# JinPLu/VeloxSeg

Hardware: AMD Instinct MI355X
Metric: training patches/s on 128^3 2-mod volumes (fwd+loss+bwd+allreduce+AdamW) (higher is better)
Workload: dtype f32

## Files before the change

### include/veloxseg_hip.h

```cpp
#ifndef VELOXSEG_HIP_H
#define VELOXSEG_HIP_H

#ifdef __cplusplus
extern "C" {
#endif

#define VX_ABI_VERSION 1

int vx_abi_version(void);
const char* vx_last_error(void);

int vx_conv3d_fwd(const float* x, const float* x2, int C1, const float* w, const float* bias, float* y,
                  int B, int Cin, int Di, int Hi, int Wi, int Cout, int K, int S, int P, int G, int ps, void* stream);
int vx_conv3d_bwd_data(const float* dy, const float* w, const float* bias_like, float* dx, float* dx2, int C1,
                       int B, int Cin, int Di, int Hi, int Wi, int Cout, int K, int S, int P, int G, int ps,
                       int accumulate, void* stream);
int vx_conv3d_bwd_weight(const float* x, const float* x2, int C1, const float* dy, float* dw, float* db,
                         int B, int Cin, int Di, int Hi, int Wi, int Cout, int K, int S, int P, int G, int ps, void* stream);

int vx_conv3d_bwd_weight_tiled(const float* x, const float* x2, int C1, const float* dy, float* dw, float* db,
                               int B, int Cin, int Di, int Hi, int Wi, int Cout, int K, int S, int P, int G, int ps, void* stream);
int vx_down_wgrad_ws_floats(int B, int Cin, int Di, int Hi, int Wi, int Cout);
int vx_down_wgrad_mfma(const float* x, const float* dy, float* dw, float* db, float* ws, long ws_floats,
                       int B, int Cin, int Di, int Hi, int Wi, int Cout, void* stream);
// ... 88 lines not shown
                 unsigned long long site2, float p2, int h16, void* stream);

int vx_jlc_tz_ok(int C, int G, int D, int H, int W);
int vx_jlc_tz_ntiles(int C, int G, int D, int H, int W);
int vx_jlc_tz_img_floats(int C, int G);
int vx_jlc_tz_set_pieces(int ns);
int vx_jlc_tz_set_min_voxels(long v);
int vx_jlc_tz_pieces(void);
int vx_jlc_tz_set_debug(int mask);
int vx_jlc_tz_prep(const float* w1, const float* w3, const float* w5, float* img, int C, int G, void* stream);
int vx_jlc_tz_fwd(const float* x, const float* img, const float* b1, const float* b3, const float* b5, float* y1, float* y3, float* y5, double* part,
                  int B, int C, int G, int D, int H, int W, void* stream);
int vx_jlc_tz_bwd(const float* g1, const float* g3, const float* g5, const float* img, const float* w1, const float* d_o, float* dx,
                  int B, int C, int G, int D, int H, int W, void* stream);
int vx_jlc_cl_ok(int C, int G, int D, int H, int W);
int vx_jlc_cl_ntiles(int C, int G, int D, int H, int W);
int vx_jlc_cl_img_floats(int C, int G);
int vx_jlc_cl_set_enabled(int on);
int vx_jlc_cl_prep(const float* w1, const float* w3, const float* w5, float* img, int C, int G, void* stream);
int vx_jlc_cl_fwd(const float* x, const float* img, const float* b1, const float* b3, const float* b5, float* y1, float* y3, float* y5, double* part,
                  int B, int C, int G, int D, int H, int W, void* stream);
int vx_jlc_cl_bwd(const float* g1, const float* g3, const float* g5, const float* img, const float* d_o, float* dx, int B, int C, int G, int D, int H, int W,
                  void* stream);
int vx_jlc_wgrad_tz_ok(int C, int G, int D, int H, int W);
int vx_jlc_wgrad_tz_set_min_voxels(long v);
int vx_jlc_wgrad_tz_set_blocks(int n);
int vx_jlc_wgrad_tz_set_spec(int on);
int vx_jlc_wgrad_tz_set_f16(int on);
int vx_jlc_wgrad_tz(const float* x, const float* g1, const float* g3, const float* g5, float* dw1, float* dw3, float* dw5, int B, int C, int G, int D, int H, int W,
                    void* stream);
int vx_jlc_tz_img_floats_ns(int C, int G, int pieces);
int vx_jlc_tz_prep_ns(const float* w1, const float* w3, const float* w5, float* img, int C, int G, int pieces, void* stream);
int vx_jlc_tz_fwd_ns(const float* x, const float* img, const float* b1, const float* b3, const float* b5, float* y1, float* y3, float* y5, double* part,
                     int B, int C, int G, int D, int H, int W, int pieces, void* stream);
int vx_jlc_tz_bwd_ns(const float* g1, const float* g3, const float* g5, const float* img, const float* w1, const float* d_o, float* dx,
                     int B, int C, int G, int D, int H, int W, int pieces, void* stream);
int vx_jlc_wgrad_tz_ns(const float* x, const float* g1, const float* g3, const float* g5, float* dw1, float* dw3, float* dw5, int B, int C, int G, int D, int H, int W,
                       int pieces, void* stream);
int vx_jlc_tz_fwd_h(const float* x, const float* img, const float* b1, const float* b3, const float* b5, void* y1, void* y3, void* y5, double* part,
                    int B, int C, int G, int D, int H, int W, int pieces, int h16, void* stream);
int vx_jlc_tz_bwd_h(const void* g1, const void* g3, const void* g5, const float* img, const float* w1, const void* d_o, float* dx,
                    int B, int C, int G, int D, int H, int W, int pieces, int h16, void* stream);
int vx_jlc_wgrad_tz_h(const float* x, const void* g1, const void* g3, const void* g5, float* dw1, float* dw3, float* dw5, int B, int C, int G, int D, int H, int W,
                      int pieces, int h16, void* stream);

int vx_in_stats(const float* x, float* stats, double* part_ws, long BC, long V, float eps, void* stream);
// ... 239 lines not shown
```

### veloxseg_amd/csrc/_vxops.cpp

```cpp
#include <torch/extension.h>
#include <torch/csrc/autograd/custom_function.h>
#include <torch/custom_class.h>
#include <torch/library.h>
#include <c10/hip/HIPStream.h>
#include <ATen/hip/impl/HIPStreamMasqueradingAsCUDA.h>
#include <ATen/hip/impl/HIPGuardImplMasqueradingAsCUDA.h>
#include <hip/hip_runtime_api.h>
#include <algorithm>
#include <map>
#include <unordered_map>
#include <tuple>
#include <functional>
#include <type_traits>
#include <memory>
#include <vector>
#include <map>
#include <tuple>
#include "../../include/veloxseg_hip.h"

using at::Tensor;
typedef c10::optional<Tensor> OptT;

namespace {

// ... 482 lines not shown
    return out;
}

void axpy_bwd_impl(AxpyState& st, const Tensor& dout_in, bool need_x_in, Tensor& dx, Tensor& dz, void* stream) {
    Tensor dout = contig(dout_in);
    const bool need_x = st.has_x && need_x_in;
    if (st.p == 0.0 && (st.alpha == 1.0 || !need_x)) { if (need_x) dx = dout; dz = dout; return; }
    if (need_x) dx = st.alpha == 1.0 ? dout : at::empty_like(dout);
    dz = st.p == 0.0 ? dout : at::empty_like(dout);
    VX(vx_axpy_drop_bwd, fp(dout), (need_x && st.alpha != 1.0) ? mp(dx) : nullptr, st.p > 0 ? mp(dz) : nullptr, (float)st.alpha, dout.numel(), st.rs,
                         (unsigned long long)st.site, (float)st.p, stream);
}

inline Tensor sum3(const Tensor& a, const Tensor& b, const Tensor& c, void* stream) {
    Tensor ac = contig(a), bc = contig(b), cc = c.defined() ? contig(c) : Tensor();
    Tensor out = at::empty_like(ac);
    VX(vx_add, fp(ac), fp(bc), fp(cc), mp(out), ac.numel(), stream);
    return out;
}

struct JLCFusedState {
    Tensor x, y, o, stats_y, stats_o;
    bool img_cl = false;
    int tz_pieces = 0;
    Tensor img;
    Tensor w1, w3, w5, b1, b3, b5, l1w, l1b, l2w, l2b;
    int B = 0, C = 0, G = 0, D = 0, H = 0, W = 0, R = 0, nch = 0;
    bool tile = false;
    bool h16 = false;
    double p = 0; int64_t site = 0; const void* rs = nullptr;
};
struct JLCState {
    std::vector<ConvState> convs;
    INState in1, in2;
    ConvState c1, c2;
    GeluState g;
    AxpyState r;
    bool fused = false;
    bool blk = false;
    JLCFusedState f;
};

struct FFNState {
    LNState ln;
    ConvState c1, c2;
    GeluState g;
// ... 369 lines not shown
    return 0;
}
static std::pair<Tensor, std::shared_ptr<JLCState>> jlc_fwd_f(const Tensor& x, const std::vector<Tensor>& ws, const std::vector<Tensor>& bs, int G, const Tensor& l1w, const Tensor& l1b, const Tensor& l2w,
                        const Tensor& l2b, double p, int64_t site, int64_t rs, int64_t stream) {
        auto st = std::make_shared<JLCState>();
        void* s_ = sp(stream);
        const int n = (int)ws.size();
        if (F.fuse_blocks && n == 3 && x.dim() == 5 && ws[0].size(2) == 1 && ws[1].size(2) == 3 && ws[2].size(2) == 5) {
            const int B = x.size(0), C = x.size(1), D = x.size(2), H = x.size(3), W = x.size(4), R = l1w.size(0);
            const long V = (long)D * H * W;
            const bool mlp_ok = vx_mlp_supported(C, R, V) && C < F.tile_min_c, tile_ok = !mlp_ok && F.jlc_tile && V % 4 == 0 && vx_inmlp_ok(C, R, V);
            if ((C / G) % 4 == 0 && (mlp_ok || tile_ok) && bs[0].defined() && bs[1].defined() && bs[2].defined()) {
                check_in(x, "jlc");
                JLCFusedState& f = st->f;
                st->blk = true;
                f.x = contig(x);
                f.w1 = ws[0]; f.w3 = ws[1]; f.w5 = ws[2]; f.b1 = bs[0]; f.b3 = bs[1]; f.b5 = bs[2]; f.l1w = l1w; f.l1b = l1b; f.l2w = l2w; f.l2b = l2b;
                f.B = B; f.C = C; f.G = G; f.D = D; f.H = H; f.W = W; f.R = R; f.p = p; f.site = site; f.rs = p > 0 ? sp(rs) : nullptr;
                const long BC = (long)B * C;
                const bool tz = F.jlc_tz && vx_jlc_tz_ok(C, G, D, H, W);
                const bool cl = !tz && F.jlc_tz && vx_jlc_cl_ok(C, G, D, H, W);
                const int nty = tz ? vx_jlc_tz_ntiles(C, G, D, H, W) : cl ? vx_jlc_cl_ntiles(C, G, D, H, W) : vx_jlc_ntiles(B, C, G, D, H, W);
                TORCH_CHECK(nty > 0, "vx_jlc_ntiles failed");
                f.nch = vx_jlc_nchunks(BC, V);
                auto dopt = f.x.options().dtype(at::kDouble);
                Tensor part_y = at::empty({3, BC, nty, 2}, dopt), part_o = at::empty({BC, (long)f.nch, 2}, dopt);
                f.tile = tile_ok;
                f.tz_pieces = tz ? vx_jlc_tz_pieces() : 0;
                f.h16 = F.act_bf16 && tz && !tile_ok && f.tz_pieces == 1 && F.jlc_wg_tz && vx_jlc_wgrad_tz_ok(C, G, D, H, W) == 1 && V > 64;
                auto iopt = f.h16 ? f.x.options().dtype(at::kBFloat16) : f.x.options();
                const long esz = f.h16 ? 2 : 4;
                f.y = at::empty({3, B, C, D, H, W}, iopt);
                char* yp = (char*)f.y.data_ptr();
                const long n1 = BC * V;
                void *y1 = yp, *y3 = yp + esz * n1, *y5 = yp + 2 * esz * n1;
                bool pre = false;
                {
                    auto it = JLC_PRE.find(f.w1.data_ptr());
                    if (it != JLC_PRE.end()) {
                        const JlcPreImg& q = it->second;
                        pre = q.C == C && q.G == G && ((tz && q.kind == 1 && q.pieces == f.tz_pieces) || (cl && q.kind == 2));
                        if (pre && q.keep) pre = q.epoch == WEIGHTS_EPOCH && q.ver == jlc_wver(f.w1, f.w3, f.w5);
                        if (pre) f.img = q.img;
                        if (!(pre && q.keep)) JLC_PRE.erase(it);
                    }
                }
                if (tz) {
                    if (!pre) {
                        f.img = at::empty({(long)vx_jlc_tz_img_floats_ns(C, G, f.tz_pieces)}, f.x.options());
                        VX(vx_jlc_tz_prep_ns, fp(f.w1), fp(f.w3), fp(f.w5), mp(f.img), C, G, f.tz_pieces, s_);
                    }
                    VX(vx_jlc_tz_fwd_h, fp(f.x), fp(f.img), fp(f.b1), fp(f.b3), fp(f.b5), y1, y3, y5, part_y.data_ptr<double>(), B, C, G, D, H, W, f.tz_pieces, (int)f.h16, s_);
                } else if (cl) {
                    f.img_cl = true;
                    if (!pre) {
                        f.img = at::empty({(long)vx_jlc_cl_img_floats(C, G)}, f.x.options());
                        VX(vx_jlc_cl_prep, fp(f.w1), fp(f.w3), fp(f.w5), mp(f.img), C, G, s_);
                    }
                    VX(vx_jlc_cl_fwd, fp(f.x), fp(f.img), fp(f.b1), fp(f.b3), fp(f.b5), (float*)y1, (float*)y3, (float*)y5, part_y.data_ptr<double>(), B, C, G, D, H, W, s_);
                } else
                VX(vx_jlc_conv_fwd, fp(f.x), fp(f.w1), fp(f.w3), fp(f.w5), fp(f.b1), fp(f.b3), fp(f.b5), (float*)y1, (float*)y3, (float*)y5, part_y.data_ptr<double>(), B, C, G, D, H, W, s_);
                f.stats_y = at::empty({3, BC, 2}, f.x.options());
                f.stats_o = at::empty({BC, 2}, f.x.options());
                f.o = at::empty(f.x.sizes(), iopt);
                VX(vx_jlc_mid_fwd_h, fp(f.x), (const void*)y1, (const void*)y3, (const void*)y5, part_y.data_ptr<double>(), nty, mp(f.stats_y), f.o.data_ptr(), part_o.data_ptr<double>(), BC, V, (float)F.in_eps, (int)f.h16, s_);
                Tensor out = at::empty_like(f.x);
                if (tile_ok) VX(vx_inmlp_fwd, fp(f.o), part_o.data_ptr<double>(), f.nch, mp(f.stats_o), fp(l1w), fp(l1b), fp(l2w), fp(l2b), mp(out), B, C, R, V, (float)F.in_eps,
                                f.rs, (unsigned long long)site, (float)p, s_);
                else
                VX(vx_mlp_fwd_h, (const void*)f.o.data_ptr(), 0, part_o.data_ptr<double>(), f.nch, mp(f.stats_o), nullptr, nullptr, fp(l1w), fp(l1b), fp(l2w), fp(l2b), mp(out), B, C, R, V,
                               (float)F.in_eps, f.rs, 0ull, 0.0f, (unsigned long long)site, (float)p, (int)f.h16, s_);
                return {out, st};
            }
        }
        st->convs.resize(n);
        std::vector<Tensor> ys;
        for (int k = 0; k < n; ++k) {
            const int K = ws[k].size(2);
            ys.push_back(conv_fwd_impl(st->convs[k], x, Tensor(), ws[k], bs[k], K, 1, K / 2, G, 1, x.requires_grad(), s_));
        }
        Tensor o = in_fwd_impl(st->in1, x, true, ys, s_);
        Tensor nrm = in_fwd_impl(st->in2, Tensor(), false, {o}, s_);
        st->fused = pw_gelu_fusable(nrm, l1w) && l2w.size(1) % 4 == 0;
        Tensor h;
        if (st->fused) h = pw_gelu_fwd_impl(st->c1, st->g, nrm, l1w, l1b, 0.0, 0, nullptr, s_);
        else {
            Tensor a = conv_fwd_impl(st->c1, nrm, Tensor(), l1w, l1b, 1, 1, 0, 1, 1, true, s_);
// ... 16 lines not shown
            const int B = f.B, C = f.C, G = f.G, D = f.D, H = f.H, W = f.W, R = f.R;
            const long V = (long)D * H * W, BC = (long)B * C, n1 = BC * V;
            const int npd = f.tile ? vx_inmlp_tiles(V) : vx_mlp_bwd_nparts(B, C, V);
            auto iopt = f.h16 ? f.x.options().dtype(at::kBFloat16) : f.x.options();
            const long esz = f.h16 ? 2 : 4;
            const int h16 = f.h16 ? 1 : 0;
            Tensor dn = at::empty(f.x.sizes(), iopt), part_dn = at::empty({BC, (long)npd, 2}, f.x.options());
            if (f.tile) {
                Tensor sc_n = at::empty_like(f.x), sc_dz = at::empty_like(f.x), sc_h = at::empty({B, R, D, H, W}, f.x.options()), sc_da = at::empty({B, R, D, H, W}, f.x.options());
                VX(vx_inmlp_bwd, fp(f.o), fp(f.stats_o), fp(f.l1w), fp(f.l1b), fp(f.l2w), fp(dout), mp(dn), mp(part_dn), mp(sc_n), mp(sc_h), mp(sc_da), mp(sc_dz), B, C, R, V,
                                 f.rs, (unsigned long long)f.site, (float)f.p, s_);
                float *dw1 = grad_ptr(f.l1w), *db1 = grad_ptr(f.l1b), *dw2 = grad_ptr(f.l2w), *db2 = grad_ptr(f.l2b);
                wgrad_submit(s_, f.x.device().index(), [=](void* s) {
                    const void* ptrs[8] = {fp(sc_h), fp(sc_dz), dw2, db2, fp(sc_n), fp(sc_da), dw1, db1};
                    const long dims[8] = {R, C, V, B, C, R, V, B};
                    VX(vx_pw_wgrad_group, ptrs, dims, 2, nullptr, nullptr, 0, s);
                });
            } else
            VX(vx_mlp_bwd_h, (const void*)f.o.data_ptr(), 0, fp(f.stats_o), nullptr, nullptr, fp(f.l1w), fp(f.l1b), fp(f.l2w), fp(dout), dn.data_ptr(), mp(part_dn), nullptr, nullptr,
                           grad_ptr(f.l1w), grad_ptr(f.l1b), grad_ptr(f.l2w), grad_ptr(f.l2b), B, C, R, V, (float)F.in_eps, f.rs, 0ull, 0.0f,
                           (unsigned long long)f.site, (float)f.p, h16, s_);
            const char* yp = (const char*)f.y.data_ptr();
            const void *y1 = yp, *y3 = yp + esz * n1, *y5 = yp + 2 * esz * n1;
            Tensor d_o = at::empty(f.x.sizes(), iopt), part_t = at::empty({3, BC, (long)f.nch, 2}, f.x.options());
            VX(vx_jlc_mid_bwd_h, fp(dout), (const void*)dn.data_ptr(), fp(part_dn), npd, (const void*)f.o.data_ptr(), fp(f.stats_o), y1, y3, y5, fp(f.stats_y), d_o.data_ptr(), mp(part_t), BC, V, h16, s_);
            Tensor g = at::empty({3, B, C, D, H, W}, iopt);
            char* gp = (char*)g.data_ptr();
            void *g1 = gp, *g3 = gp + esz * n1, *g5 = gp + 2 * esz * n1;
            VX(vx_jlc_gk_h, (const void*)d_o.data_ptr(), y1, y3, y5, fp(f.stats_y), fp(part_t), g1, g3, g5, BC, V, h16, s_);
            Tensor dx;
            if (need_x) {
                dx = f.h16 ? at::empty_like(f.x) : dn;
                if (f.img.defined() && f.img_cl) VX(vx_jlc_cl_bwd, (const float*)g1, (const float*)g3, (const float*)g5, fp(f.img), fp(d_o), mp(dx), B, C, G, D, H, W, s_);
                else if (f.img.defined()) VX(vx_jlc_tz_bwd_h, (const void*)g1, (const void*)g3, (const void*)g5, fp(f.img), fp(f.w1), (const void*)d_o.data_ptr(), mp(dx), B, C, G, D, H, W, f.tz_pieces, h16, s_);
                else
                VX(vx_jlc_conv_bwd, (const float*)g1, (const float*)g3, (const float*)g5, fp(f.w1), fp(f.w3), fp(f.w5), fp(d_o), mp(dx), B, C, G, D, H, W, s_);
            }
            grad_ptr(f.b1); grad_ptr(f.b3); grad_ptr(f.b5);
            const int Cg = C / G;
            {
                Tensor xk = f.x, gk = g;
                float* dw1 = f.w1.requires_grad() ? grad_ptr(f.w1) : nullptr;
                float* dw3 = f.w3.requires_grad() ? grad_ptr(f.w3) : nullptr;
                float* dw5 = f.w5.requires_grad() ? grad_ptr(f.w5) : nullptr;
                const bool g1fast = F.use_gconv1 && (Cg == 4 || Cg == 8 || Cg == 16) && V % 4 == 0;
                const bool tzok = F.jlc_wg_tz && dw1 && dw3 && dw5 && vx_jlc_wgrad_tz_ok(C, G, D, H, W);
                const bool wga = F.jlc_wg_tz && dw1 && dw3 && dw5 && vx_jlc_wgrad_gather_ok(C, G, D, H, W) == 1 && (!tzok || V <= 64);
                const bool wtz = !wga && tzok;
                const int wg_pieces = f.tz_pieces ? f.tz_pieces : vx_jlc_tz_pieces();
                wgrad_submit(s_, f.x.device().index(), [=](void* s) {
                    if (h16) {
                        const char* gh = (const char*)gk.data_ptr();
                        TORCH_CHECK(wtz, "veloxseg_amd.jlc: the 16-bit g_k of the bf16 storage mode need the matrix-pipe weight-gradient kernel");
                        VX(vx_jlc_wgrad_tz_h, fp(xk), (const void*)gh, (const void*)(gh + 2 * n1), (const void*)(gh + 4 * n1), dw1, dw3, dw5, B, C, G, D, H, W, wg_pieces, 1, s);
                        return;
                    }
                    const float* gq = gk.data_ptr<float>();
                    if (wga) {
                        VX(vx_jlc_wgrad_gather, fp(xk), gq, gq + n1, gq + 2 * n1, dw1, dw3, dw5, B, C, G, D, H, W, s);
// ... 548 lines not shown
        for (auto& r : PROF.recs) {
            float ms = 0.0f;
            hipEventElapsedTime(&ms, r.e0, r.e1);
            hipEventDestroy(r.e0); hipEventDestroy(r.e1);
            py::tuple key(r.key.size());
            for (size_t i = 0; i < r.key.size(); ++i) key[i] = py::int_(r.key[i]);
            out.append(py::make_tuple(std::string(r.name), key, ms));
        }
        PROF.recs.clear();
        return out;
    });
    m.def("set_conv_mfma", [](bool on) { F.use_conv_mfma = on; });
    m.def("set_bf16_expand", [](bool on) { F.bf16_expand = on; });
    m.def("get_bf16_expand", []() { return F.bf16_expand; });
    m.def("set_expand_split", [](int64_t ns) { F.expand_split = (ns == 2 || ns == 3 || ns == 22) ? (int)ns : 0; });
    m.def("get_expand_split", []() { return F.expand_split; });
    m.def("set_tile_min_c", [](int64_t c) { F.tile_min_c = (int)c; });
    m.def("set_act_bf16", [](bool on) { F.act_bf16 = on; }, "bf16 STORAGE mode: block-internal tensors of the JLC blocks / full-resolution heads and their gradients as bf16 arrays (with set_bf16_expand and vx_jlc_tz_set_pieces(1): functional.set_precision('bf16'))");
    m.def("get_act_bf16", []() { return F.act_bf16; });
    m.def("set_upconv_wgrad_mfma", [](bool on) { F.upconv_wgrad_mfma = on; });
    m.def("set_jlc_tz", [](bool on) { F.jlc_tz = on; });
    m.def("get_jlc_tz", []() { return F.jlc_tz; });
    m.def("set_jlc_wg_tz", [](bool on) { F.jlc_wg_tz = on; });
    m.def("set_jlc_tile", [](bool on) { F.jlc_tile = on; });
    m.def("set_expand_wgrad_split", [](bool on) { F.expand_wgrad_split = on; });
    m.def("set_fuse_blocks", [](bool on) { F.fuse_blocks = on; });
    m.def("set_fuse_bwd_add", [](bool on) { F.fuse_bwd_add = on; });
    m.def("set_fuse_res", [](bool on) { F.fuse_res = on; });
    m.def("set_in_split2", [](bool on) { F.in_split2 = on; });
    m.def("set_skip_in_bias", [](bool on) { F.skip_in_bias = on; });

    m.def("conv_fwd", [](const Tensor& x, const OptT& x2, const Tensor& w, const OptT& b, int K, int S, int P, int G, int ps, int64_t stream) {
        auto st = std::make_shared<ConvState>();
        Tensor y = conv_fwd_impl(*st, x, x2.value_or(Tensor()), w, b.value_or(Tensor()), K, S, P, G, ps, x.requires_grad(), sp(stream));
        return py::make_tuple(y, st);
    });
    m.def("conv_bwd", [](std::shared_ptr<ConvState> st, const Tensor& dy, bool need_x, int64_t stream) {
        Tensor dx, dx2;
        conv_bwd_impl(*st, dy, need_x, dx, dx2, sp(stream));
        return py::make_tuple(dx.defined() ? py::cast(dx) : py::none(), dx2.defined() ? py::cast(dx2) : py::none());
    });

    m.def("in_fwd", [](const OptT& res, bool act, const std::vector<Tensor>& ys, int64_t stream) {
        auto st = std::make_shared<INState>();
        Tensor out = in_fwd_impl(*st, res.value_or(Tensor()), act, ys, sp(stream));
        return py::make_tuple(out, st);
// ... 51 lines not shown
```

### veloxseg_amd/csrc/jlc_cl.hip

```cpp
#include "vx_common.h"
#include <stdlib.h>
#include "../../include/veloxseg_hip.h"

typedef _Float16 cl_h8 __attribute__((ext_vector_type(8)));
typedef _Float16 cl_h2 __attribute__((ext_vector_type(2)));
typedef float cl_f2 __attribute__((ext_vector_type(2)));
typedef float cl_f4 __attribute__((ext_vector_type(4)));
typedef uint32_t cl_u4 __attribute__((ext_vector_type(4)));
#define CL_MFMA(a, b, c) __builtin_amdgcn_mfma_f32_16x16x32_f16(__builtin_bit_cast(cl_h8, (a)), __builtin_bit_cast(cl_h8, (b)), (c), 0, 0, 0)

__device__ __forceinline__ void cl_split2(float a, float b, uint32_t& hi, uint32_t& lo) {
    const cl_f2 v = {a, b};
    const cl_h2 h = __builtin_convertvector(v, cl_h2);
    const cl_h2 l = __builtin_convertvector(v - __builtin_convertvector(h, cl_f2), cl_h2);
    hi = __builtin_bit_cast(uint32_t, h);
    lo = __builtin_bit_cast(uint32_t, l);
}
__device__ __forceinline__ int cl_exp16(float m) {
    if (!(m > 0.0f) || !(m < 3.0e38f)) return 0;
    int e = 13 - ilogbf(m);
    return e > 100 ? 100 : (e < -100 ? -100 : e);
}

struct ClTaps { signed char od[128], oh[128], ow[128]; unsigned char k5[128], k3[128]; };
// ... 357 lines not shown
    if (C / G == 8) { if (tpw == 2) CL_F(8, 2) else CL_F(8, 1) }
    else { if (tpw == 2) CL_F(16, 2) else CL_F(16, 1) }
#undef CL_F
    VX_LAUNCH_CHECK("vx_jlc_cl_fwd");
    return 0;
}
extern "C" int vx_jlc_cl_bwd(const float* g1, const float* g3, const float* g5, const float* img, const float* d_o, float* dx, int B, int C, int G, int D, int H, int W,
                             void* stream) {
    VX_REQUIRE(g1 && g3 && g5 && img && dx, "vx_jlc_cl_bwd: null pointer");
    VxCl p; int tpw; size_t sf, sb;
    if (!cl_plan(p, B, C, G, D, H, W, tpw, sf, sb)) VX_FAIL(-3, "vx_jlc_cl_bwd: shape not covered (C=%d G=%d %dx%dx%d)", C, G, D, H, W);
    hipStream_t st = (hipStream_t)stream;
    const dim3 grid((unsigned)p.nchunk, (unsigned)(B * G));
    const float* esc = cl_esc(const_cast<float*>(img), C, G);
    const cl_u4* im = reinterpret_cast<const cl_u4*>(img);
#define CL_B(CG_, T_) { static bool once = false; if (!once) { cl_attr(vx_jlc_cl_bwd_k<CG_, T_>); once = true; } \
        vx_jlc_cl_bwd_k<CG_, T_><<<grid, dim3(256), sb, st>>>(g1, g3, g5, im, esc, d_o, dx, p); }
    if (C / G == 8) { if (tpw == 2) CL_B(8, 2) else CL_B(8, 1) }
    else { if (tpw == 2) CL_B(16, 2) else CL_B(16, 1) }
#undef CL_B
    VX_LAUNCH_CHECK("vx_jlc_cl_bwd");
    return 0;
}
```

Before: 1067.

## Fuse JLC channel-last conv with instance-norm mid stage into single-block kernels

Adds fused forward and backward kernels for small JLC volumes (V up to 256/512 voxels). Each block handles one (batch, group) pair and keeps the whole group in LDS. In the forward pass, the grouped 1/3/5 conv via split-f16 MFMA, the bias add and the norm statistics/normalization run in one launch. In the backward pass, the mid-stage backward, the gk gradients and the data-gradient conv are merged into one kernel, which drops the intermediate d_o tensor, the part_t buffer and several launches. The cost is a grid of only B*G blocks of 512 threads plus large LDS use, so occupancy on deep low-resolution layers may be poor.

```diff
diff --git a/include/veloxseg_hip.h b/include/veloxseg_hip.h
--- a/include/veloxseg_hip.h
+++ b/include/veloxseg_hip.h
@@ -134,6 +134,13 @@
                   int B, int C, int G, int D, int H, int W, void* stream);
 int vx_jlc_cl_bwd(const float* g1, const float* g3, const float* g5, const float* img, const float* d_o, float* dx, int B, int C, int G, int D, int H, int W,
                   void* stream);
+int vx_jlc_cl_set_fused(int on);
+int vx_jlc_cl_fused_ok(int C, int G, int D, int H, int W);
+int vx_jlc_cl_fused_fwd(const float* x, const float* img, const float* b1, const float* b3, const float* b5, float* y1, float* y3, float* y5, float* stats_y,
+                        float* o, double* part_o, int B, int C, int G, int D, int H, int W, float eps, void* stream);
+int vx_jlc_cl_fused_bwd(const float* dout, const float* dn, const float* part_dn, int npd, const float* o, const float* stats_o, const float* y1, const float* y3,
+                        const float* y5, const float* stats_y, const float* img, float* g1, float* g3, float* g5, float* dx, int B, int C, int G, int D, int H,
+                        int W, void* stream);
 int vx_jlc_wgrad_tz_ok(int C, int G, int D, int H, int W);
 int vx_jlc_wgrad_tz_set_min_voxels(long v);
 int vx_jlc_wgrad_tz_set_blocks(int n);
diff --git a/veloxseg_amd/csrc/_vxops.cpp b/veloxseg_amd/csrc/_vxops.cpp
--- a/veloxseg_amd/csrc/_vxops.cpp
+++ b/veloxseg_amd/csrc/_vxops.cpp
@@ -528,6 +528,7 @@
 struct JLCFusedState {
     Tensor x, y, o, stats_y, stats_o;
     bool img_cl = false;
+    bool cl_fused = false;
     int tz_pieces = 0;
     Tensor img;
     Tensor w1, w3, w5, b1, b3, b5, l1w, l1b, l2w, l2b;
@@ -943,7 +944,8 @@
                 const bool cl = !tz && F.jlc_tz && vx_jlc_cl_ok(C, G, D, H, W);
                 const int nty = tz ? vx_jlc_tz_ntiles(C, G, D, H, W) : cl ? vx_jlc_cl_ntiles(C, G, D, H, W) : vx_jlc_ntiles(B, C, G, D, H, W);
                 TORCH_CHECK(nty > 0, "vx_jlc_ntiles failed");
-                f.nch = vx_jlc_nchunks(BC, V);
+                f.cl_fused = cl && vx_jlc_cl_fused_ok(C, G, D, H, W) == 1;
+                f.nch = f.cl_fused ? 1 : vx_jlc_nchunks(BC, V);
                 auto dopt = f.x.options().dtype(at::kDouble);
                 Tensor part_y = at::empty({3, BC, nty, 2}, dopt), part_o = at::empty({BC, (long)f.nch, 2}, dopt);
                 f.tile = tile_ok;
@@ -978,12 +980,15 @@
                         f.img = at::empty({(long)vx_jlc_cl_img_floats(C, G)}, f.x.options());
                         VX(vx_jlc_cl_prep, fp(f.w1), fp(f.w3), fp(f.w5), mp(f.img), C, G, s_);
                     }
-                    VX(vx_jlc_cl_fwd, fp(f.x), fp(f.img), fp(f.b1), fp(f.b3), fp(f.b5), (float*)y1, (float*)y3, (float*)y5, part_y.data_ptr<double>(), B, C, G, D, H, W, s_);
+                    if (!f.cl_fused) VX(vx_jlc_cl_fwd, fp(f.x), fp(f.img), fp(f.b1), fp(f.b3), fp(f.b5), (float*)y1, (float*)y3, (float*)y5, part_y.data_ptr<double>(), B, C, G, D, H, W, s_);
                 } else
                 VX(vx_jlc_conv_fwd, fp(f.x), fp(f.w1), fp(f.w3), fp(f.w5), fp(f.b1), fp(f.b3), fp(f.b5), (float*)y1, (float*)y3, (float*)y5, part_y.data_ptr<double>(), B, C, G, D, H, W, s_);
                 f.stats_y = at::empty({3, BC, 2}, f.x.options());
                 f.stats_o = at::empty({BC, 2}, f.x.options());
                 f.o = at::empty(f.x.sizes(), iopt);
+                if (f.cl_fused) VX(vx_jlc_cl_fused_fwd, fp(f.x), fp(f.img), fp(f.b1), fp(f.b3), fp(f.b5), (float*)y1, (float*)y3, (float*)y5, mp(f.stats_y), mp(f.o), part_o.data_ptr<double>(),
+                                   B, C, G, D, H, W, (float)F.in_eps, s_);
+                else
                 VX(vx_jlc_mid_fwd_h, fp(f.x), (const void*)y1, (const void*)y3, (const void*)y5, part_y.data_ptr<double>(), nty, mp(f.stats_y), f.o.data_ptr(), part_o.data_ptr<double>(), BC, V, (float)F.in_eps, (int)f.h16, s_);
                 Tensor out = at::empty_like(f.x);
                 if (tile_ok) VX(vx_inmlp_fwd, fp(f.o), part_o.data_ptr<double>(), f.nch, mp(f.stats_o), fp(l1w), fp(l1b), fp(l2w), fp(l2b), mp(out), B, C, R, V, (float)F.in_eps,
@@ -1046,19 +1051,25 @@
                            (unsigned long long)f.site, (float)f.p, h16, s_);
             const char* yp = (const char*)f.y.data_ptr();
             const void *y1 = yp, *y3 = yp + esz * n1, *y5 = yp + 2 * esz * n1;
-            Tensor d_o = at::empty(f.x.sizes(), iopt), part_t = at::empty({3, BC, (long)f.nch, 2}, f.x.options());
-            VX(vx_jlc_mid_bwd_h, fp(dout), (const void*)dn.data_ptr(), fp(part_dn), npd, (const void*)f.o.data_ptr(), fp(f.stats_o), y1, y3, y5, fp(f.stats_y), d_o.data_ptr(), mp(part_t), BC, V, h16, s_);
             Tensor g = at::empty({3, B, C, D, H, W}, iopt);
             char* gp = (char*)g.data_ptr();
             void *g1 = gp, *g3 = gp + esz * n1, *g5 = gp + 2 * esz * n1;
+            Tensor dx;
+            if (f.cl_fused) {
+                if (need_x) dx = at::empty_like(f.x);
+                VX(vx_jlc_cl_fused_bwd, fp(dout), fp(dn), fp(part_dn), npd, fp(f.o), fp(f.stats_o), (const float*)y1, (const float*)y3, (const float*)y5, fp(f.stats_y), fp(f.img),
+                   (float*)g1, (float*)g3, (float*)g5, need_x ? mp(dx) : nullptr, B, C, G, D, H, W, s_);
+            } else {
+            Tensor d_o = at::empty(f.x.sizes(), iopt), part_t = at::empty({3, BC, (long)f.nch, 2}, f.x.options());
+            VX(vx_jlc_mid_bwd_h, fp(dout), (const void*)dn.data_ptr(), fp(part_dn), npd, (const void*)f.o.data_ptr(), fp(f.stats_o), y1, y3, y5, fp(f.stats_y), d_o.data_ptr(), mp(part_t), BC, V, h16, s_);
             VX(vx_jlc_gk_h, (const void*)d_o.data_ptr(), y1, y3, y5, fp(f.stats_y), fp(part_t), g1, g3, g5, BC, V, h16, s_);
-            Tensor dx;
             if (need_x) {
                 dx = f.h16 ? at::empty_like(f.x) : dn;
                 if (f.img.defined() && f.img_cl) VX(vx_jlc_cl_bwd, (const float*)g1, (const float*)g3, (const float*)g5, fp(f.img), fp(d_o), mp(dx), B, C, G, D, H, W, s_);
                 else if (f.img.defined()) VX(vx_jlc_tz_bwd_h, (const void*)g1, (const void*)g3, (const void*)g5, fp(f.img), fp(f.w1), (const void*)d_o.data_ptr(), mp(dx), B, C, G, D, H, W, f.tz_pieces, h16, s_);
                 else
                 VX(vx_jlc_conv_bwd, (const float*)g1, (const float*)g3, (const float*)g5, fp(f.w1), fp(f.w3), fp(f.w5), fp(d_o), mp(dx), B, C, G, D, H, W, s_);
+            }
             }
             grad_ptr(f.b1); grad_ptr(f.b3); grad_ptr(f.b5);
             const int Cg = C / G;
@@ -1653,6 +1664,7 @@
     m.def("set_jlc_tz", [](bool on) { F.jlc_tz = on; });
     m.def("get_jlc_tz", []() { return F.jlc_tz; });
     m.def("set_jlc_wg_tz", [](bool on) { F.jlc_wg_tz = on; });
+    m.def("set_jlc_cl_fused", [](bool on) { vx_jlc_cl_set_fused(on ? 1 : 0); });
     m.def("set_jlc_tile", [](bool on) { F.jlc_tile = on; });
     m.def("set_expand_wgrad_split", [](bool on) { F.expand_wgrad_split = on; });
     m.def("set_fuse_blocks", [](bool on) { F.fuse_blocks = on; });
diff --git a/veloxseg_amd/csrc/jlc_cl.hip b/veloxseg_amd/csrc/jlc_cl.hip
--- a/veloxseg_amd/csrc/jlc_cl.hip
+++ b/veloxseg_amd/csrc/jlc_cl.hip
@@ -1,5 +1,7 @@
 #include "vx_common.h"
 #include <stdlib.h>
+#include <algorithm>
+#include <type_traits>
 #include "../../include/veloxseg_hip.h"
 
 typedef _Float16 cl_h8 __attribute__((ext_vector_type(8)));
@@ -403,3 +405,423 @@
     VX_LAUNCH_CHECK("vx_jlc_cl_bwd");
     return 0;
 }
+
+constexpr int CLF_NW = 8, CLF_NTHR = CLF_NW * 64, CLF_DEPTH = 8;
+constexpr int CLF_F_X = 1024;
+constexpr int CLF_B_RED = 1024, CLF_B_X = 2048;
+
+struct ClfGeo { const unsigned char* xs[3]; int lo[3]; const int* toff[3]; int sgn[3]; };
+template <int CG, int TPW, int C, int E0, int E1, class Flush>
+__device__ __forceinline__ void clf_part(cl_u4 (&fh)[CLF_DEPTH], cl_u4 (&fl)[CLF_DEPTH], const cl_u4* __restrict__ ig, const ClfGeo& q, const int (&hp)[3][TPW], int Gl, Flush&& flush) {
+    using KK = ClK<CG>;
+    constexpr int NA = TPW == 1 ? 3 : 1;
+    cl_f4 acc[TPW][NA];
+#pragma unroll
+    for (int t = 0; t < TPW; ++t)
+#pragma unroll
+        for (int a = 0; a < NA; ++a) acc[t][a] = (cl_f4){0.f, 0.f, 0.f, 0.f};
+    const int* __restrict__ tf = q.toff[C];
+    const unsigned char* __restrict__ xc = q.xs[C];
+    const int lo = q.lo[C], sgn = q.sgn[C];
+    auto tapoff = [&](int e) -> int {
+        e = e < E0 ? E0 : (e > E1 - 1 ? E1 - 1 : e);
+        const int s = C == 0 ? e : C == 1 ? e - KK::NS5 : KK::S1;
+        return sgn * tf[CG == 8 ? 4 * s + Gl : 2 * s + (Gl >> 1)];
+    };
+    constexpr int EB0 = E0 / CLF_DEPTH * CLF_DEPTH;
+    int offn[CLF_DEPTH];
+#pragma unroll
+    for (int j = 0; j < CLF_DEPTH; ++j) offn[j] = tapoff(EB0 + j);
+    cl_u4 nbh[TPW], nbl[TPW];
+#pragma unroll
+    for (int t = 0; t < TPW; ++t) {
+        nbh[t] = *reinterpret_cast<const cl_u4*>(xc + offn[0] + hp[C][t]);
+        nbl[t] = *reinterpret_cast<const cl_u4*>(xc + offn[0] + lo + hp[C][t]);
+    }
+#pragma unroll 1
+    for (int eb = EB0; eb < E1; eb += CLF_DEPTH) {
+        int off[CLF_DEPTH];
+#pragma unroll
+        for (int j = 0; j < CLF_DEPTH; ++j) off[j] = offn[j];
+#pragma unroll
+        for (int j = 0; j < CLF_DEPTH; ++j) offn[j] = tapoff(eb + CLF_DEPTH + j);
+#pragma unroll
+        for (int j = 0; j < CLF_DEPTH; ++j) {
+            const int e = eb + j;
+            cl_u4 bh[TPW], bl[TPW];
+#pragma unroll
+            for (int t = 0; t < TPW; ++t) { bh[t] = nbh[t]; bl[t] = nbl[t]; }
+            const int on = j + 1 < CLF_DEPTH ? off[j + 1 < CLF_DEPTH ? j + 1 : 0] : offn[0];
+#pragma unroll
+            for (int t = 0; t < TPW; ++t) {
+                nbh[t] = *reinterpret_cast<const cl_u4*>(xc + on + hp[C][t]);
+                nbl[t] = *reinterpret_cast<const cl_u4*>(xc + on + lo + hp[C][t]);
+            }
+            __builtin_amdgcn_sched_barrier(0);
+            if (e >= E0 && e < E1) {
+                const cl_u4 ah = fh[j], al = fl[j];
+                if (e + CLF_DEPTH < KK::NE) { fh[j] = ig[(long)(e + CLF_DEPTH) * 128]; fl[j] = ig[(long)(e + CLF_DEPTH) * 128 + 64]; }
+#pragma unroll
+                for (int t = 0; t < TPW; ++t) {
+                    acc[t][0] = CL_MFMA(ah, bh[t], acc[t][0]);
+                    acc[t][NA == 3 ? 1 : 0] = CL_MFMA(ah, bl[t], acc[t][NA == 3 ? 1 : 0]);
+                    acc[t][NA == 3 ? 2 : 0] = CL_MFMA(al, bh[t], acc[t][NA == 3 ? 2 : 0]);
+                }
+            }
+            __builtin_amdgcn_sched_barrier(0);
+        }
+    }
+    cl_f4 res[TPW];
+#pragma unroll
+    for (int t = 0; t < TPW; ++t) res[t] = NA == 3 ? acc[t][0] + (acc[t][1] + acc[t][NA - 1]) : acc[t][0];
+    flush(std::integral_constant<int, C>{}, res);
+}
+template <int CG, int TPW, class Flush>
+__device__ __forceinline__ void clf_stream(const cl_u4* __restrict__ ig, const ClfGeo& q, const int (&hp)[3][TPW], int Gl, Flush&& flush) {
+    using KK = ClK<CG>;
+    cl_u4 fh[CLF_DEPTH], fl[CLF_DEPTH];
+#pragma unroll
+    for (int j = 0; j < CLF_DEPTH; ++j) { fh[j] = ig[j * 128]; fl[j] = ig[j * 128 + 64]; }
+    clf_part<CG, TPW, 0, 0, KK::NS5>(fh, fl, ig, q, hp, Gl, flush);
+    clf_part<CG, TPW, 1, KK::NS5, KK::NS5 + KK::NS3>(fh, fl, ig, q, hp, Gl, flush);
+    clf_part<CG, TPW, 2, KK::NS5 + KK::NS3, KK::NE>(fh, fl, ig, q, hp, Gl, flush);
+}
+template <int CG>
+__device__ __forceinline__ int clf_stage(unsigned char* __restrict__ dst, const float* __restrict__ src, const VxCl& p, const ClHalo& hl, float* __restrict__ red) {
+    constexpr int NH = CG / 8;
+    float mx = 0.0f;
+    for (int i = threadIdx.x; i < CG * p.V; i += CLF_NTHR) mx = fmaxf(mx, fabsf(src[i]));
+    mx = vx_wave_max(mx);
+    if ((threadIdx.x & 63) == 0) red[threadIdx.x >> 6] = mx;
+    const int nz = 2 * NH * hl.npos;
+    for (int i = threadIdx.x; i < nz; i += CLF_NTHR) reinterpret_cast<cl_u4*>(dst)[i] = (cl_u4){0u, 0u, 0u, 0u};
+    __syncthreads();
+    const int e = cl_exp16(fmaxf(fmaxf(fmaxf(red[0], red[1]), fmaxf(red[2], red[3])), fmaxf(fmaxf(red[4], red[5]), fmaxf(red[6], red[7]))));
+    const float sc = ldexpf(1.0f, e);
+    for (int i = threadIdx.x; i < NH * p.V; i += CLF_NTHR) {
+        const int half = i / p.V, v = i - half * p.V;
+        const int w = v % p.W, hh = (v / p.W) % p.H, d = v / (p.W * p.H);
+        float x[8];
+#pragma unroll
+        for (int j = 0; j < 8; ++j) x[j] = src[(long)(8 * half + j) * p.V + v] * sc;
+        uint32_t h[4], l[4];
+#pragma unroll
+        for (int q = 0; q < 4; ++q) cl_split2(x[2 * q], x[2 * q + 1], h[q], l[q]);
+        const int hp = ((d + hl.P) * hl.HH + (hh + hl.P)) * hl.HW + (w + hl.P);
+        reinterpret_cast<cl_u4*>(dst)[half * hl.npos + hp] = (cl_u4){h[0], h[1], h[2], h[3]};
+        reinterpret_cast<cl_u4*>(dst)[(NH + half) * hl.npos + hp] = (cl_u4){l[0], l[1], l[2], l[3]};
+    }
+    return e;
+}
+
+template <int CG, int TPW>
+__global__ void __launch_bounds__(CLF_NTHR) vx_jlc_cl_fused_fwd_k(const float* __restrict__ x, const cl_u4* __restrict__ img, const float* __restrict__ esc,
+                                                                  const float* __restrict__ b1, const float* __restrict__ b3, const float* __restrict__ b5,
+                                                                  float* __restrict__ y1, float* __restrict__ y3, float* __restrict__ y5, float* __restrict__ stats_y,
+                                                                  float* __restrict__ out_o, double* __restrict__ part_o, float eps, VxCl p) {
+    using KK = ClK<CG>;
+    extern __shared__ __attribute__((aligned(16))) unsigned char cl_lds[];
+    int* __restrict__ toff = reinterpret_cast<int*>(cl_lds);
+    float* __restrict__ red = reinterpret_cast<float*>(cl_lds + 512);
+    unsigned char* __restrict__ xs = cl_lds + CLF_F_X;
+    const int bg = blockIdx.x, b = bg / p.G, g = bg - b * p.G;
+    const int tid = threadIdx.x, lane = tid & 63, wave = tid >> 6, n = lane & 15, Gl = lane >> 4;
+    for (int i = tid; i < 128; i += CLF_NTHR) toff[i] = ((cl_taps.od[i] * p.h5.HH + cl_taps.oh[i]) * p.h5.HW + cl_taps.ow[i]) * 16;
+    const int ex = clf_stage<CG>(xs, x + ((long)b * p.C + (long)g * CG) * p.V, p, p.h5, red);
+    __syncthreads();
+    int hp[3][TPW], pv[TPW];
+#pragma unroll
+    for (int t = 0; t < TPW; ++t) {
+        const int tile = wave * TPW + t;
+        const int v = 16 * tile + n;
+        pv[t] = (tile < p.NT && v < p.V) ? v : -1;
+        const int vc = v < p.V ? v : p.V - 1;
+        const int w = vc % p.W, hh = (vc / p.W) % p.H, d = vc / (p.W * p.H);
+        hp[0][t] = (((d + 2) * p.h5.HH + (hh + 2)) * p.h5.HW + (w + 2)) * 16;
+        hp[1][t] = hp[0][t]; hp[2][t] = hp[0][t];
+    }
+    cl_f4 yv[3][TPW];
+#pragma unroll
+    for (int t = 0; t < TPW; ++t) { yv[0][t] = (cl_f4){0.f, 0.f, 0.f, 0.f}; yv[1][t] = yv[0][t]; yv[2][t] = yv[0][t]; }
+    if (wave * TPW < p.NT) {
+        ClfGeo q;
+        q.xs[0] = xs + (CG == 16 ? (Gl & 1) : 0) * p.h5.npos * 16; q.lo[0] = KK::NH * p.h5.npos * 16; q.toff[0] = toff; q.sgn[0] = 1;
+        q.xs[1] = q.xs[2] = q.xs[0]; q.lo[1] = q.lo[2] = q.lo[0]; q.toff[1] = q.toff[2] = toff; q.sgn[1] = q.sgn[2] = 1;
+        clf_stream<CG, TPW>(img + ((long)g * KK::NE) * 128 + lane, q, hp, Gl, [&](auto c, cl_f4 (&a)[TPW]) {
+#pragma unroll
+            for (int t = 0; t < TPW; ++t) yv[2 - decltype(c)::value][t] = a[t];
+        });
+    }
+    const float f5 = ldexpf(1.0f, -(ex + (int)esc[g * 3 + 0])), f3 = ldexpf(1.0f, -(ex + (int)esc[g * 3 + 1])), f1 = ldexpf(1.0f, -(ex + (int)esc[g * 3 + 2]));
+    const long BC = (long)p.B * p.C;
+    const int V = p.V, cb = b * p.C + g * CG;
+    float* __restrict__ ybuf = reinterpret_cast<float*>(xs);
+    __syncthreads();
+    if (4 * Gl < CG) {
+#pragma unroll
+        for (int i = 0; i < 4; ++i) {
+            const int cl = 4 * Gl + i, co = g * CG + cl;
+            const float c1 = b1 ? b1[co] : 0.0f, c3 = b3 ? b3[co] : 0.0f, c5 = b5 ? b5[co] : 0.0f;
+#pragma unroll
+            for (int t = 0; t < TPW; ++t)
+                if (pv[t] >= 0) {
+                    ybuf[(0 * CG + cl) * V + pv[t]] = fmaf(yv[0][t][i], f1, c1);
+                    ybuf[(1 * CG + cl) * V + pv[t]] = fmaf(yv[1][t][i], f3, c3);
+                    ybuf[(2 * CG + cl) * V + pv[t]] = fmaf(yv[2][t][i], f5, c5);
+                }
+        }
+    }
+    __syncthreads();
+    constexpr int NCW = CG / 8, NITM = 8 / NCW;
+    float* __restrict__ yo[3] = {y1, y3, y5};
+#pragma unroll
+    for (int cc = 0; cc < NCW; ++cc) {
+        const int cl = wave + 8 * cc;
+        const long base = ((long)cb + cl) * V;
+        float yk[NITM][3], xv[NITM];
+        float s[3] = {0.f, 0.f, 0.f}, q[3] = {0.f, 0.f, 0.f};
+#pragma unroll
+        for (int it = 0; it < NITM; ++it) {
+            const int v = it * 64 + lane;
+            xv[it] = v < V ? x[base + v] : 0.0f;
+#pragma unroll
+            for (int k = 0; k < 3; ++k) {
+                const float val = v < V ? ybuf[(k * CG + cl) * V + v] : 0.0f;
+                yk[it][k] = val;
+                if (v < V) yo[k][base + v] = val;
+                s[k] += val; q[k] = fmaf(val, val, q[k]);
+            }
+        }
+        float mk[3], rk[3];
+#pragma unroll
+        for (int k = 0; k < 3; ++k) {
+            const double sd = vx_wave_sum((double)s[k]), qd = vx_wave_sum((double)q[k]);
+            const double m = sd / (double)V;
+            double var = qd / (double)V - m * m;
+            var = var < 0.0 ? 0.0 : var;
+            mk[k] = (float)m; rk[k] = (float)(1.0 / sqrt(var + (double)eps));
+            if (lane == 0) { stats_y[((long)k * BC + cb + cl) * 2] = mk[k]; stats_y[((long)k * BC + cb + cl) * 2 + 1] = rk[k]; }
+        }
+        float so = 0.0f, qo = 0.0f;
+#pragma unroll
+        for (int it = 0; it < NITM; ++it) {
+            const int v = it * 64 + lane;
+            if (v < V) {
+                const float ov = xv[it] + vx_gelu_fast((yk[it][0] - mk[0]) * rk[0]) + vx_gelu_fast((yk[it][1] - mk[1]) * rk[1]) + vx_gelu_fast((yk[it][2] - mk[2]) * rk[2]);
+                out_o[base + v] = ov;
+                so += ov; qo = fmaf(ov, ov, qo);
+            }
+        }
+        const double sd = vx_wave_sum((double)so), qd = vx_wave_sum((double)qo);
+        if (lane == 0) { part_o[((long)cb + cl) * 2] = sd; part_o[((long)cb + cl) * 2 + 1] = qd; }
+    }
+}
+
+__device__ __forceinline__ void clf_put(unsigned char* __restrict__ dst, int npos, int NH, int c, int hp, float v) {
+    const _Float16 h = (_Float16)v;
+    const _Float16 l = (_Float16)(v - (float)h);
+    const int half = c >> 3, j = c & 7;
+    *reinterpret_cast<_Float16*>(dst + ((size_t)(half * npos + hp) * 16 + 2 * j)) = h;
+    *reinterpret_cast<_Float16*>(dst + ((size_t)((NH + half) * npos + hp) * 16 + 2 * j)) = l;
+}
+
+template <int CG, int TPW>
+__global__ void __launch_bounds__(CLF_NTHR) vx_jlc_cl_fused_bwd_k(const float* __restrict__ dout, const float* __restrict__ dn, const float* __restrict__ part_dn, int npd,
+                                                                  const float* __restrict__ o_, const float* __restrict__ stats_o, const float* __restrict__ y1,
+                                                                  const float* __restrict__ y3, const float* __restrict__ y5, const float* __restrict__ stats_y,
+                                                                  const cl_u4* __restrict__ img, const float* __restrict__ esc, float* __restrict__ g1, float* __restrict__ g3,
+                                                                  float* __restrict__ g5, float* __restrict__ dx, VxCl p) {
+    using KK = ClK<CG>;
+    constexpr int NCW = CG / 8, NITM = 8 / NCW;
+    extern __shared__ __attribute__((aligned(16))) unsigned char cl_lds[];
+    int* __restrict__ toff5 = reinterpret_cast<int*>(cl_lds);
+    int* __restrict__ toff3 = toff5 + 128;
+    float* __restrict__ red = reinterpret_cast<float*>(cl_lds + CLF_B_RED);
+    const int sz5 = 2 * KK::NH * p.h5.npos * 16, sz3 = 2 * KK::NH * p.h3.npos * 16, sz1 = 2 * KK::NH * p.h1.npos * 16;
+    unsigned char* __restrict__ x5 = cl_lds + CLF_B_X;
+    unsigned char* __restrict__ x3 = x5 + sz5;
+    unsigned char* __restrict__ x1 = x3 + sz3;
+    float* __restrict__ dos = reinterpret_cast<float*>(x1 + sz1);
+    const int bg = blockIdx.x, b = bg / p.G, g = bg - b * p.G;
+    const int tid = threadIdx.x, lane = tid & 63, wave = tid >> 6, n = lane & 15, Gl = lane >> 4;
+    const int V = p.V, cb = b * p.C + g * CG;
+    const long BC = (long)p.B * p.C;
+    for (int i = tid; i < 128; i += CLF_NTHR) {
+        toff5[i] = ((cl_taps.od[i] * p.h5.HH + cl_taps.oh[i]) * p.h5.HW + cl_taps.ow[i]) * 16;
+        toff3[i] = ((cl_taps.od[i] * p.h3.HH + cl_taps.oh[i]) * p.h3.HW + cl_taps.ow[i]) * 16;
+    }
+    for (int i = tid; i < (sz5 + sz3 + sz1) / 16; i += CLF_NTHR) reinterpret_cast<cl_u4*>(x5)[i] = (cl_u4){0u, 0u, 0u, 0u};
+    float tk[8][3], yh[8][3];
+    float mx[3] = {0.f, 0.f, 0.f};
+#pragma unroll
+    for (int cc = 0; cc < NCW; ++cc) {
+        const int cl = wave + 8 * cc;
+        const long bc = (long)cb + cl;
+        float ds = 0.0f, dq = 0.0f;
+        for (int i = lane; i < npd; i += 64) { ds += part_dn[(bc * npd + i) * 2]; dq += part_dn[(bc * npd + i) * 2 + 1]; }
+        ds = vx_wave_sum(ds); dq = vx_wave_sum(dq);
+        const float dm1 = ds / (float)V, dm2 = dq / (float)V;
+        const float mo = stats_o[2 * bc], ro = stats_o[2 * bc + 1];
+        float mk[3], rk[3];
+#pragma unroll
+        for (int k = 0; k < 3; ++k) { mk[k] = stats_y[((long)k * BC + bc) * 2]; rk[k] = stats_y[((long)k * BC + bc) * 2 + 1]; }
+        float sum[6] = {0.f, 0.f, 0.f, 0.f, 0.f, 0.f};
+#pragma unroll
+        for (int it = 0; it < NITM; ++it) {
+            const int u = cc * NITM + it, v = it * 64 + lane;
+#pragma unroll
+            for (int k = 0; k < 3; ++k) { tk[u][k] = 0.0f; yh[u][k] = 0.0f; }
+            if (v < V) {
+                const long idx = bc * V + v;
+                const float yk[3] = {y1[idx], y3[idx], y5[idx]};
+                const float nh = (o_[idx] - mo) * ro;
+                const float d = dout[idx] + ro * (dn[idx] - dm1 - nh * dm2);
+                dos[cl * V + v] = d;
+#pragma unroll
+                for (int k = 0; k < 3; ++k) {
+                    const float yy = (yk[k] - mk[k]) * rk[k];
+                    const float t = d * vx_gelu_grad_fast(yy);
+                    sum[2 * k] += t;
+                    sum[2 * k + 1] = fmaf(t, yy, sum[2 * k + 1]);
+                    tk[u][k] = t; yh[u][k] = yy;
+                }
+            }
+        }
+#pragma unroll
+        for (int e = 0; e < 6; ++e) sum[e] = vx_wave_sum(sum[e]) / (float)V;
+#pragma unroll
+        for (int it = 0; it < NITM; ++it) {
+            const int u = cc * NITM + it, v = it * 64 + lane;
+            if (v < V) {
+                const long idx = bc * V + v;
+#pragma unroll
+                for (int k = 0; k < 3; ++k) {
+                    const float gk = rk[k] * (tk[u][k] - sum[2 * k] - yh[u][k] * sum[2 * k + 1]);
+                    tk[u][k] = gk;
+                    mx[k] = fmaxf(mx[k], fabsf(gk));
+                }
+                g1[idx] = tk[u][0]; g3[idx] = tk[u][1]; g5[idx] = tk[u][2];
+            }
+        }
+    }
+    if (dx == nullptr) return;
+#pragma unroll
+    for (int k = 0; k < 3; ++k) { mx[k] = vx_wave_max(mx[k]); if (lane == 0) red[wave * 3 + k] = mx[k]; }
+    __syncthreads();
+    int ek[3];
+#pragma unroll
+    for (int k = 0; k < 3; ++k) {
+        float m = 0.0f;
+        for (int w = 0; w < CLF_NW; ++w) m = fmaxf(m, red[w * 3 + k]);
+        ek[k] = cl_exp16(m);
+    }
+    {
+        const float s1 = ldexpf(1.0f, ek[0]), s3 = ldexpf(1.0f, ek[1]), s5 = ldexpf(1.0f, ek[2]);
+#pragma unroll
+        for (int cc = 0; cc < NCW; ++cc)
+#pragma unroll
+            for (int it = 0; it < NITM; ++it) {
+                const int u = cc * NITM + it, v = it * 64 + lane, cl = wave + 8 * cc;
+                if (v < V) {
+                    const int w = v % p.W, hh = (v / p.W) % p.H, d = v / (p.W * p.H);
+                    clf_put(x5, p.h5.npos, KK::NH, cl, ((d + 2) * p.h5.HH + (hh + 2)) * p.h5.HW + (w + 2), tk[u][2] * s5);
+                    clf_put(x3, p.h3.npos, KK::NH, cl, ((d + 1) * p.h3.HH + (hh + 1)) * p.h3.HW + (w + 1), tk[u][1] * s3);
+                    clf_put(x1, p.h1.npos, KK::NH, cl, (d * p.h1.HH + hh) * p.h1.HW + w, tk[u][0] * s1);
+                }
+            }
+    }
+    __syncthreads();
+    const int hsel = CG == 16 ? (Gl & 1) : 0;
+    int hp[3][TPW], pv[TPW];
+#pragma unroll
+    for (int t = 0; t < TPW; ++t) {
+        const int tile = wave * TPW + t;
+        const int v = 16 * tile + n;
+        pv[t] = (tile < p.NT && v < V) ? v : -1;
+        const int vc = v < V ? v : V - 1;
+        const int w = vc % p.W, hh = (vc / p.W) % p.H, d = vc / (p.W * p.H);
+        hp[0][t] = (((d + 2) * p.h5.HH + (hh + 2)) * p.h5.HW + (w + 2)) * 16;
+        hp[1][t] = (((d + 1) * p.h3.HH + (hh + 1)) * p.h3.HW + (w + 1)) * 16;
+        hp[2][t] = ((d * p.h1.HH + hh) * p.h1.HW + w) * 16;
+    }
+    cl_f4 tot[TPW];
+#pragma unroll
+    for (int t = 0; t < TPW; ++t) tot[t] = (cl_f4){0.f, 0.f, 0.f, 0.f};
+    if (wave * TPW < p.NT) {
+        const float f5 = ldexpf(1.0f, -(ek[2] + (int)esc[g * 3 + 0])), f3 = ldexpf(1.0f, -(ek[1] + (int)esc[g * 3 + 1])), f1 = ldexpf(1.0f, -(ek[0] + (int)esc[g * 3 + 2]));
+        ClfGeo q;
+        q.xs[0] = x5 + hsel * p.h5.npos * 16; q.lo[0] = KK::NH * p.h5.npos * 16; q.toff[0] = toff5; q.sgn[0] = -1;
+        q.xs[1] = x3 + hsel * p.h3.npos * 16; q.lo[1] = KK::NH * p.h3.npos * 16; q.toff[1] = toff3; q.sgn[1] = -1;
+        q.xs[2] = x1 + hsel * p.h1.npos * 16; q.lo[2] = KK::NH * p.h1.npos * 16; q.toff[2] = toff3; q.sgn[2] = 0;
+        clf_stream<CG, TPW>(img + ((long)(p.G + g) * KK::NE) * 128 + lane, q, hp, Gl, [&](auto c, cl_f4 (&a)[TPW]) {
+            const float f = decltype(c)::value == 0 ? f5 : decltype(c)::value == 1 ? f3 : f1;
+#pragma unroll
+            for (int t = 0; t < TPW; ++t) tot[t] += a[t] * f;
+        });
+    }
+    if (4 * Gl < CG) {
+#pragma unroll
+        for (int t = 0; t < TPW; ++t)
+#pragma unroll
+            for (int i = 0; i < 4; ++i)
+                if (pv[t] >= 0) {
+                    const int cl = 4 * Gl + i;
+                    dx[((long)cb + cl) * V + pv[t]] = tot[t][i] + dos[cl * V + pv[t]];
+                }
+    }
+}
+
+static int g_cl_fused = 1;
+static bool clf_plan(VxCl& p, int B, int C, int G, int D, int H, int W, int& tpw, size_t& shm_f, size_t& shm_b) {
+    int t0; size_t a, c;
+    if (!cl_plan(p, B, C, G, D, H, W, t0, a, c)) return false;
+    const int CG = C / G;
+    if (p.V > (CG == 8 ? 512 : 256)) return false;
+    const int per = (p.NT + CLF_NW - 1) / CLF_NW;
+    tpw = per <= 1 ? 1 : per <= 2 ? 2 : 4;
+    const size_t nh = CG / 8;
+    shm_f = CLF_F_X + std::max<size_t>(2 * nh * p.h5.npos * 16, (size_t)3 * CG * p.V * 4);
+    shm_b = CLF_B_X + 2 * nh * ((size_t)p.h5.npos + p.h3.npos + p.h1.npos) * 16 + (size_t)CG * p.V * 4;
+    return shm_f <= 160 * 1024 && shm_b <= 160 * 1024;
+}
+extern "C" int vx_jlc_cl_set_fused(int on) { g_cl_fused = on ? 1 : 0; return 0; }
+extern "C" int vx_jlc_cl_fused_ok(int C, int G, int D, int H, int W) {
+    VxCl p; int tpw; size_t sf, sb;
+    return (g_cl_fused && clf_plan(p, 1, C, G, D, H, W, tpw, sf, sb)) ? 1 : 0;
+}
+extern "C" int vx_jlc_cl_fused_fwd(const float* x, const float* img, const float* b1, const float* b3, const float* b5, float* y1, float* y3, float* y5, float* stats_y,
+                                   float* o, double* part_o, int B, int C, int G, int D, int H, int W, float eps, void* stream) {
+    VX_REQUIRE(x && img && y1 && y3 && y5 && stats_y && o && part_o, "vx_jlc_cl_fused_fwd: null pointer");
+    VxCl p; int tpw; size_t sf, sb;
+    if (!clf_plan(p, B, C, G, D, H, W, tpw, sf, sb)) VX_FAIL(-3, "vx_jlc_cl_fused_fwd: shape not covered (C=%d G=%d %dx%dx%d)", C, G, D, H, W);
+    hipStream_t st = (hipStream_t)stream;
+    const dim3 grid((unsigned)(B * G));
+    const float* esc = cl_esc(const_cast<float*>(img), C, G);
+    const cl_u4* im = reinterpret_cast<const cl_u4*>(img);
+#define CLF_F(CG_, T_) { static bool once = false; if (!once) { cl_attr(vx_jlc_cl_fused_fwd_k<CG_, T_>); once = true; } \
+        vx_jlc_cl_fused_fwd_k<CG_, T_><<<grid, dim3(CLF_NTHR), sf, st>>>(x, im, esc, b1, b3, b5, y1, y3, y5, stats_y, o, part_o, eps, p); }
+    if (C / G == 8) { if (tpw == 4) CLF_F(8, 4) else if (tpw == 2) CLF_F(8, 2) else CLF_F(8, 1) }
+    else { if (tpw == 2) CLF_F(16, 2) else CLF_F(16, 1) }
+#undef CLF_F
+    VX_LAUNCH_CHECK("vx_jlc_cl_fused_fwd");
+    return 0;
+}
+extern "C" int vx_jlc_cl_fused_bwd(const float* dout, const float* dn, const float* part_dn, int npd, const float* o, const float* stats_o, const float* y1, const float* y3,
+                                   const float* y5, const float* stats_y, const float* img, float* g1, float* g3, float* g5, float* dx, int B, int C, int G, int D, int H,
+                                   int W, void* stream) {
+    VX_REQUIRE(dout && dn && part_dn && npd > 0 && o && stats_o && y1 && y3 && y5 && stats_y && img && g1 && g3 && g5, "vx_jlc_cl_fused_bwd: bad args");
+    VX_REQUIRE(dx != dn && dx != dout, "vx_jlc_cl_fused_bwd: dx must not alias an input");
+    VxCl p; int tpw; size_t sf, sb;
+    if (!clf_plan(p, B, C, G, D, H, W, tpw, sf, sb)) VX_FAIL(-3, "vx_jlc_cl_fused_bwd: shape not covered (C=%d G=%d %dx%dx%d)", C, G, D, H, W);
+    hipStream_t st = (hipStream_t)stream;
+    const dim3 grid((unsigned)(B * G));
+    const float* esc = cl_esc(const_cast<float*>(img), C, G);
+    const cl_u4* im = reinterpret_cast<const cl_u4*>(img);
+#define CLF_B(CG_, T_) { static bool once = false; if (!once) { cl_attr(vx_jlc_cl_fused_bwd_k<CG_, T_>); once = true; } \
+        vx_jlc_cl_fused_bwd_k<CG_, T_><<<grid, dim3(CLF_NTHR), sb, st>>>(dout, dn, part_dn, npd, o, stats_o, y1, y3, y5, stats_y, im, esc, g1, g3, g5, dx, p); }
+    if (C / G == 8) { if (tpw == 4) CLF_B(8, 4) else if (tpw == 2) CLF_B(8, 2) else CLF_B(8, 1) }
+    else { if (tpw == 2) CLF_B(16, 2) else CLF_B(16, 1) }
+#undef CLF_B
+    VX_LAUNCH_CHECK("vx_jlc_cl_fused_bwd");
+    return 0;
+}
```

Result: no change. 1078, median of 6 (+1.0%).
